# ChenFengYe/motion-latent-diffusion

Hardware: NVIDIA H100
Metric: motions/sec @ 50-step DDIM text-to-motion, batch 256 (higher is better)
Workload: dtype f16x2-split (fp32-equivalent, fp32 accumulate)

## Files before the change

### mld_b200/csrc/engine.cu

```cuda
#include "engine.h"

#include <math.h>
#include <string.h>

#include <algorithm>

#include "gemm_tc.h"
#include "misc_kernels.cuh"

static thread_local std::string g_err;
void mldb_set_err(const std::string& s) { g_err = s; }
extern "C" const char* mldb_last_error(void) { return g_err.c_str(); }
extern "C" int mldb_abi_version(void) { return MLDB_ABI_VERSION; }

extern "C" void mldb_default_config(mldb_config* c) {
  memset(c, 0, sizeof *c);
  c->abi_version = MLDB_ABI_VERSION;
  c->cond_kind = MLDB_COND_TEXT;
  c->arch = MLDB_ARCH_TRANS_ENC;
  c->latent_dim = 256; c->n_lat = 1; c->num_heads = 4; c->ff_size = 1024; c->num_layers = 9;
  c->text_dim = 768; c->nclasses = 12; c->nfeats = 263; c->diffusion_only = 0;
  c->flip_sin_to_cos = 1; c->freq_shift = 0.0f; c->guidance_scale = 7.5f;
  c->vae_kind = MLDB_VAE_MLD; c->vae_layers = 9; c->vae_heads = 4; c->vae_ff = 1024;
  c->vae_nfeats = 263;
// ... 379 lines not shown
  env = getenv("MLDB_BRANCHES");
  if (env) h->branches = std::min(std::max(atoi(env), 1), (int)mldb_handle::MAX_BRANCHES);
  e = cudaEventCreateWithFlags(&h->ev_fork, cudaEventDisableTiming);
  for (int i = 0; i < mldb_handle::MAX_BRANCHES - 1 && e == cudaSuccess; ++i) {
    e = cudaStreamCreateWithFlags(&h->br_stream[i], cudaStreamNonBlocking);
    if (e == cudaSuccess) e = cudaEventCreateWithFlags(&h->ev_join[i], cudaEventDisableTiming);
  }
  if (e != cudaSuccess) { mldb_destroy(h); FAIL(MLDB_ERR_CUDA, "branch streams: %s", cudaGetErrorString(e)); }
  for (int i = 0; i < mldb_handle::MAX_BRANCHES && e == cudaSuccess; ++i) {
    e = cudaMalloc((void**)&h->ffn_scratch[i], TC_FFN_SCRATCH_BYTES);
    if (e == cudaSuccess) e = cudaMalloc((void**)&h->ffn_flags[i], TC_FFN_FLAG_BYTES);
    if (e == cudaSuccess) e = cudaMemset(h->ffn_flags[i], 0, TC_FFN_FLAG_BYTES);
  }
  if (e != cudaSuccess) { mldb_destroy(h); FAIL(MLDB_ERR_CUDA, "ffn scratch: %s", cudaGetErrorString(e)); }
  env = getenv("MLDB_FFN_SPLIT");
  if (env) tc_set_ffn_split(h->tc, atoi(env) != 0);
  env = getenv("MLDB_FFN_FUSED");
  if (env) tc_set_ffn_fused(h->tc, atoi(env) != 0);
  *out = h;
  return MLDB_OK;
}

extern "C" void mldb_destroy(mldb_handle* h) {
  if (!h) return;
  DeviceGuard guard(h->device);
  cudaDeviceSynchronize();
  for (auto& kv : h->plans) {
    if (kv.second->exec) cudaGraphExecDestroy(kv.second->exec);
    delete kv.second;
  }
  for (void* p : h->allocs) cudaFree(p);
  if (h->cap_stream) cudaStreamDestroy(h->cap_stream);
  for (int i = 0; i < mldb_handle::MAX_BRANCHES - 1; ++i) {
    if (h->br_stream[i]) cudaStreamDestroy(h->br_stream[i]);
    if (h->ev_join[i]) cudaEventDestroy(h->ev_join[i]);
  }
  if (h->ev_fork) cudaEventDestroy(h->ev_fork);
  for (int i = 0; i < mldb_handle::MAX_BRANCHES; ++i) { cudaFree(h->ffn_scratch[i]); cudaFree(h->ffn_flags[i]); }
  mldb_comm_release(h);
  tc_destroy(h->tc);
  delete h;
}

extern "C" int mldb_set_option(mldb_handle* h, const char* name, const char* value) {
  if (!h || !name || !value) FAIL(MLDB_ERR_INVALID, "null argument");
  if (!strcmp(name, "gemm")) {
    if (!strcmp(value, "tc")) h->use_tc = true;
    else if (!strcmp(value, "simt")) h->use_tc = false;
    else FAIL(MLDB_ERR_INVALID, "gemm must be tc|simt");
  } else if (!strcmp(name, "ffn_fused")) {
    tc_set_ffn_fused(h->tc, atoi(value) != 0);
  } else if (!strcmp(name, "ffn_split")) {
    tc_set_ffn_split(h->tc, atoi(value) != 0);
  } else if (!strcmp(name, "attn")) {
    if (!strcmp(value, "tc")) h->attn_kind = 0;
    else if (!strcmp(value, "mma")) h->attn_kind = 1;
    else if (!strcmp(value, "simt")) h->attn_kind = 2;
    else FAIL(MLDB_ERR_INVALID, "attn must be tc|mma|simt");
  } else if (!strcmp(name, "branches")) {
    h->branches = std::min(std::max(atoi(value), 1), (int)mldb_handle::MAX_BRANCHES);
  } else if (!strcmp(name, "graph")) {
    h->use_graph = strcmp(value, "0") != 0;
  } else if (!strcmp(name, "t2m_chunk")) {
    h->t2m.chunk = std::max(atoi(value), 0);
  } else if (!strcmp(name, "a2m_chunk")) {
    h->a2m.chunk = std::max(atoi(value), 0);
  } else if (!strcmp(name, "stgcn_chunk")) {
    h->stgcn.chunk = std::max(atoi(value), 0);
  } else if (!strcmp(name, "smpl_chunk")) {
    h->smpl.chunk = std::max(atoi(value), 0);
  } else {
    FAIL(MLDB_ERR_INVALID, "unknown option %s", name);
  }
  for (auto& kv : h->plans) {
    if (kv.second->exec) { cudaGraphExecDestroy(kv.second->exec); kv.second->exec = nullptr; }
  }
  return MLDB_OK;
}

extern "C" int64_t mldb_launch_count(const mldb_handle* h) { return h ? h->launches : 0; }

extern "C" int mldb_load_tensor(mldb_handle* h, const char* key, const void* data,
                                const int64_t* shape, int32_t ndim, int32_t dtype) {
  if (!h || !key || !data || (!shape && ndim != 0)) FAIL(MLDB_ERR_INVALID, "null argument");
  if (dtype != MLDB_DTYPE_F32) FAIL(MLDB_ERR_UNSUPPORTED, "only fp32 tensors are accepted");
  if (h->finalized) FAIL(MLDB_ERR_STATE, "weights already finalized");
  auto it = h->raw.find(key);
  if (it == h->raw.end()) FAIL(MLDB_ERR_INVALID, "unexpected state-dict key '%s'", key);
  RawTensor& t = it->second;
  if ((int)t.shape.size() != ndim) FAIL(MLDB_ERR_INVALID, "key '%s': rank %d, expected %d", key, ndim, (int)t.shape.size());
  size_t n = 1;
  for (int i = 0; i < ndim; ++i) {
    if (shape[i] != t.shape[i]) FAIL(MLDB_ERR_INVALID, "key '%s': dim %d is %lld, expected %lld", key, i, (long long)shape[i], (long long)t.shape[i]);
    n *= (size_t)shape[i];
  }
  t.host.resize(n);
  DeviceGuard guard(h->device);
  CK(cudaMemcpy(t.host.data(), data, n * sizeof(float), cudaMemcpyDefault));
  t.loaded = true;
  return MLDB_OK;
}

extern "C" int mldb_finalize_weights(mldb_handle* h, void* stream) {
  (void)stream;
  if (!h) FAIL(MLDB_ERR_INVALID, "null handle");
  if (h->finalized) FAIL(MLDB_ERR_STATE, "already finalized");
// ... 228 lines not shown
```

### mld_b200/csrc/gemm_tc.cu

```cuda
#include "gemm_tc.h"

#include <algorithm>

#include "tc_common.cuh"

namespace {
using namespace tc;

constexpr int BM = 128, BK = 64;
constexpr int NUM_THREADS = 384;
constexpr int MMA_THREADS = 256;
constexpr int CONSUMER_WARPS = 8;
constexpr int MAX_N = 1024;
constexpr int MAX_N_WIDE = 4096;

struct TcParams {
  int M, N, kblocks, kb1;
  int m_tiles, n_tiles;
  float inv_scale;
  const float* bias;
  const float* addtab;
  int act;
  __half* out_hi; __half* out_lo; int ld_out, out_col0;
  float* out_f32; int ldc;
  const float* res_f32;
  int in_group, out_group, out_off;
  const int32_t* zero_lengths;
  const __half* res_hi; const __half* res_lo; int ld_res;
  const float* gamma; const float* beta;
  long long* tl;
};

enum { EPI_FAST = 0, EPI_LN = 1, EPI_GENERIC = 2, EPI_RES = 3, EPI_F32 = 4 };

template <int BN>
struct TileCfg {
  static constexpr int A_BYTES = BM * BK * 2;
  static constexpr int W_BYTES = BN * BK * 2;
  static constexpr int STAGE_BYTES = 2 * A_BYTES + 2 * W_BYTES;
  static constexpr int STAGES = BN == 256 ? 2 : 3;
  static constexpr int SMEM_BYTES = STAGES * STAGE_BYTES + 256 + 1024;
  static_assert(SMEM_BYTES <= 232448, "shared memory budget");
};

__device__ __forceinline__ void store_split2(__half* hi, __half* lo, int64_t o, float x0, float x1) {
  uint32_t h, l;
  split2(x0, x1, h, l);
  *reinterpret_cast<uint32_t*>(hi + o) = h;
  *reinterpret_cast<uint32_t*>(lo + o) = l;
}

template <int ACT, int N>
__device__ __forceinline__ void fast_group(const float (&d)[N], int j, float sc, float2 b, float (&x)[4]) {
  x[0] = fmaf(d[4 * j], sc, b.x); x[1] = fmaf(d[4 * j + 1], sc, b.y);
  x[2] = fmaf(d[4 * j + 2], sc, b.x); x[3] = fmaf(d[4 * j + 3], sc, b.y);
#pragma unroll
  for (int e = 0; e < 4; ++e) {
    if (ACT == ACT_GELU) x[e] = gelu_fast(x[e]);
    if (ACT == ACT_QUICKGELU) x[e] = quick_gelu_f(x[e]);
    if (ACT == ACT_LEAKY) x[e] = apply_act(x[e], ACT_LEAKY);
  }
}

__device__ __forceinline__ void quad_transpose(uint32_t (&v)[4], int l) {
  const bool b2 = l & 2, b1 = l & 1;
  uint32_t r0 = __shfl_xor_sync(0xffffffffu, b2 ? v[0] : v[2], 2), r1 = __shfl_xor_sync(0xffffffffu, b2 ? v[1] : v[3], 2);
  if (b2) { v[0] = r0; v[1] = r1; } else { v[2] = r0; v[3] = r1; }
  r0 = __shfl_xor_sync(0xffffffffu, b1 ? v[0] : v[1], 1); r1 = __shfl_xor_sync(0xffffffffu, b1 ? v[2] : v[3], 1);
  if (b1) { v[0] = r0; v[2] = r1; } else { v[1] = r0; v[3] = r1; }
}

template <class Load>
__device__ __forceinline__ void ring_produce(int& q_next, int total, int need, const uint64_t* bar_empty, int stages,
                                             Load&& load) {
  while (q_next < total) {
    const uint32_t bar = smem_u32(&bar_empty[q_next % stages]), par = (((uint32_t)(q_next / stages)) & 1u) ^ 1u;
    if (q_next <= need) mbar_wait(bar, par);
    else if (!__shfl_sync(0xffffffffu, (int)mbar_test(bar, par), 0)) break;
    load(q_next++);
  }
}

template <class Res, class Out>
__device__ __forceinline__ void ln_rows(float (&d)[128], float sc, const float* bias, const float* gamma,
                                        const float* beta, int cp, Res&& res, Out&& out) {
  float s0 = 0.0f, s1 = 0.0f;
#pragma unroll
  for (int j = 0; j < 32; ++j) {
    const int n = 8 * j + cp;
    const float2 b = bias ? __ldg(reinterpret_cast<const float2*>(bias + n)) : make_float2(0.0f, 0.0f);
    float x[4] = {fmaf(d[4 * j], sc, b.x), fmaf(d[4 * j + 1], sc, b.y), fmaf(d[4 * j + 2], sc, b.x),
                  fmaf(d[4 * j + 3], sc, b.y)};
    res(j, x);
    d[4 * j] = x[0]; d[4 * j + 1] = x[1]; d[4 * j + 2] = x[2]; d[4 * j + 3] = x[3];
    s0 += x[0] + x[1]; s1 += x[2] + x[3];
  }
  const float mean0 = quad_sum(s0) * (1.0f / 256), mean1 = quad_sum(s1) * (1.0f / 256);
  float q0 = 0.0f, q1 = 0.0f;
#pragma unroll
  for (int j = 0; j < 32; ++j) {
    const float a0 = d[4 * j] - mean0, a1 = d[4 * j + 1] - mean0, a2 = d[4 * j + 2] - mean1, a3 = d[4 * j + 3] - mean1;
    d[4 * j] = a0; d[4 * j + 1] = a1; d[4 * j + 2] = a2; d[4 * j + 3] = a3;
    q0 = fmaf(a0, a0, fmaf(a1, a1, q0));
    q1 = fmaf(a2, a2, fmaf(a3, a3, q1));
  }
  const float rstd0 = rsqrtf(quad_sum(q0) * (1.0f / 256) + 1e-5f), rstd1 = rsqrtf(quad_sum(q1) * (1.0f / 256) + 1e-5f);
#pragma unroll
  for (int j = 0; j < 32; ++j) {
    const int n = 8 * j + cp;
    const float2 g = __ldg(reinterpret_cast<const float2*>(gamma + n)), be = __ldg(reinterpret_cast<const float2*>(beta + n));
    const float y[4] = {fmaf(d[4 * j] * rstd0, g.x, be.x), fmaf(d[4 * j + 1] * rstd0, g.y, be.y),
                        fmaf(d[4 * j + 2] * rstd1, g.x, be.x), fmaf(d[4 * j + 3] * rstd1, g.y, be.y)};
    out(j, y);
  }
}

__device__ __forceinline__ void ln_epilogue(float (&d)[128], float sc, const float* bias, const __half* res_hi,
                                            const __half* res_lo, int ld_res, const float* gamma, const float* beta,
                                            __half* out_hi, __half* out_lo, int ld_out, int r_lo, int M, int cp) {
  const bool ok0 = r_lo < M, ok1 = r_lo + 8 < M;
  ln_rows(d, sc, bias, gamma, beta, cp,
          [&](int j, float (&x)[4]) {
            if (!res_hi) return;
            const int n = 8 * j + cp;
            if (ok0) {
              const int64_t o = (int64_t)r_lo * ld_res + n;
              const float2 h = __half22float2(*reinterpret_cast<const __half2*>(res_hi + o));
              const float2 l = __half22float2(*reinterpret_cast<const __half2*>(res_lo + o));
              x[0] = (x[0] + h.x) + l.x; x[1] = (x[1] + h.y) + l.y;
            }
            if (ok1) {
              const int64_t o = (int64_t)(r_lo + 8) * ld_res + n;
              const float2 h = __half22float2(*reinterpret_cast<const __half2*>(res_hi + o));
              const float2 l = __half22float2(*reinterpret_cast<const __half2*>(res_lo + o));
              x[2] = (x[2] + h.x) + l.x; x[3] = (x[3] + h.y) + l.y;
            }
          },
          [&](int j, const float (&y)[4]) {
            const int n = 8 * j + cp;
            if (ok0) store_split2(out_hi, out_lo, (int64_t)r_lo * ld_out + n, y[0], y[1]);
            if (ok1) store_split2(out_hi, out_lo, (int64_t)(r_lo + 8) * ld_out + n, y[2], y[3]);
          });
}

__device__ __forceinline__ void ln_tile(float (&d)[128], float sc, const float* bias, const float* gamma,
                                        const float* beta, uint8_t* tile, int rl, int lane, int cp) {
  uint8_t* const row0 = tile + rl * 128 + cp * 2;
  const int sw = lane >> 2;
  auto at = [&](int j, int h, int plane) {
    return reinterpret_cast<__half2*>(row0 + plane * 65536 + h * 1024 + (j >> 3) * 16384 + (((j & 7) ^ sw) << 4));
  };
  ln_rows(d, sc, bias, gamma, beta, cp,
          [&](int j, float (&x)[4]) {
#pragma unroll
            for (int h = 0; h < 2; ++h) {
              const float2 hi = __half22float2(*at(j, h, 0)), lo = __half22float2(*at(j, h, 1));
              x[2 * h] = (x[2 * h] + hi.x) + lo.x; x[2 * h + 1] = (x[2 * h + 1] + hi.y) + lo.y;
            }
          },
          [&](int j, const float (&y)[4]) {
#pragma unroll
            for (int h = 0; h < 2; ++h) {
              uint32_t hi, lo;
              split2(y[2 * h], y[2 * h + 1], hi, lo);
              *reinterpret_cast<uint32_t*>(at(j, h, 0)) = hi;
              *reinterpret_cast<uint32_t*>(at(j, h, 1)) = lo;
            }
          });
}

template <int BN, int EPI, int ACT = ACT_NONE>
__global__ void __launch_bounds__(NUM_THREADS, 1)
k_gemm_tc(const __grid_constant__ CUtensorMap tmA1h, const __grid_constant__ CUtensorMap tmA1l,
          const __grid_constant__ CUtensorMap tmA2h, const __grid_constant__ CUtensorMap tmA2l,
          const __grid_constant__ CUtensorMap tmWh, const __grid_constant__ CUtensorMap tmWl, const TcParams p) {
  static_assert(EPI != EPI_LN || BN == 256, "the LayerNorm epilogue covers a full 256-wide row");
  using Cfg = TileCfg<BN>;
  constexpr int STAGES = Cfg::STAGES;
  extern __shared__ uint8_t smem_raw[];
  uint8_t* smem = smem_raw + smem_pad1024(smem_raw);
  uint64_t* bar_full = reinterpret_cast<uint64_t*>(smem + STAGES * Cfg::STAGE_BYTES);
  uint64_t* bar_empty = bar_full + STAGES;

  const int warp = __shfl_sync(0xffffffffu, (int)(threadIdx.x >> 5), 0), lane = threadIdx.x & 31;
  int tl_n = 0;
  tl_event(p.tl, tl_n, 40);
  const int ntiles = p.m_tiles * p.n_tiles;
  const int nlocal = (ntiles - (int)blockIdx.x + (int)gridDim.x - 1) / (int)gridDim.x;
  auto decode = [&](int j, int& m0, int& n0) {
    const int t = (int)blockIdx.x + j * (int)gridDim.x;
    m0 = (t / p.n_tiles) * BM;
    n0 = (t % p.n_tiles) * BN;
  };

  if (threadIdx.x == 0) {
    for (int s = 0; s < STAGES; ++s) {
      mbar_init(smem_u32(&bar_full[s]), 1);
      mbar_init(smem_u32(&bar_empty[s]), CONSUMER_WARPS);
    }
    asm volatile("fence.mbarrier_init.release.cluster;" ::: "memory");
    tma_prefetch_desc(&tmA1h); tma_prefetch_desc(&tmA1l); tma_prefetch_desc(&tmWh); tma_prefetch_desc(&tmWl);
  }
  pdl_trigger();
  __syncthreads();
  pdl_wait();
  tl_event(p.tl, tl_n, 41);

  if (warp < 4) {
    reg_dec<40>();
    if (warp != 0) return;
    int kbg = 0;
    for (int j = 0; j < nlocal; ++j) {
      int m0, n0;
      decode(j, m0, n0);
      tl_event(p.tl, tl_n, 1, j);
      for (int kb = 0; kb < p.kblocks; ++kb, ++kbg) {
        const int s = kbg % STAGES;
        mbar_wait(smem_u32(&bar_empty[s]), (((uint32_t)(kbg / STAGES)) & 1u) ^ 1u);
        if (elect_one()) {
          if (kb == 0 && j + 1 < nlocal) {
            int m1, n1;
            decode(j + 1, m1, n1);
            if (m1 != m0) {
              for (int k2 = 0; k2 < p.kblocks; ++k2) {
                if (k2 < p.kb1) { tma_prefetch_2d(&tmA1h, k2 * BK, m1); tma_prefetch_2d(&tmA1l, k2 * BK, m1); }
                else { tma_prefetch_2d(&tmA2h, (k2 - p.kb1) * BK, m1); tma_prefetch_2d(&tmA2l, (k2 - p.kb1) * BK, m1); }
              }
            }
          }
          const uint32_t full = smem_u32(&bar_full[s]);
          mbar_expect_tx(full, Cfg::STAGE_BYTES);
          const uint32_t sAh = smem_u32(smem + s * Cfg::STAGE_BYTES), sAl = sAh + Cfg::A_BYTES;
          const uint32_t sWh = sAl + Cfg::A_BYTES, sWl = sWh + Cfg::W_BYTES;
          if (kb < p.kb1) {
            tma_load_2d(sAh, &tmA1h, full, kb * BK, m0);
            tma_load_2d(sAl, &tmA1l, full, kb * BK, m0);
          } else {
            tma_load_2d(sAh, &tmA2h, full, (kb - p.kb1) * BK, m0);
            tma_load_2d(sAl, &tmA2l, full, (kb - p.kb1) * BK, m0);
          }
          tma_load_2d(sWh, &tmWh, full, kb * BK, n0);
          tma_load_2d(sWl, &tmWl, full, kb * BK, n0);
        }
        __syncwarp();
      }
    }
    return;
  }
  reg_inc<232>();
  const int cw = (warp >> 2) - 1;
  const int cp = 2 * (lane & 3);
  float d[BN / 2];
  int kbg = 0;
  for (int it = 0; it < nlocal; ++it) {
    int m0, n0;
    decode(it, m0, n0);
    tl_event(p.tl, tl_n, 2, it);
    for (int kb = 0; kb < p.kblocks; ++kb, ++kbg) {
      const int s = kbg % STAGES;
      mbar_wait(smem_u32(&bar_full[s]), ((uint32_t)(kbg / STAGES)) & 1u);
      const uint32_t sAh = smem_u32(smem + s * Cfg::STAGE_BYTES) + cw * (64 * 128), sAl = sAh + Cfg::A_BYTES;
      const uint32_t sWh = smem_u32(smem + s * Cfg::STAGE_BYTES) + 2 * Cfg::A_BYTES, sWl = sWh + Cfg::W_BYTES;
      wg_fence();
      kblock_ss<BN>(d, sAh, sAl, sWh, sWl, kb == 0);
      wg_commit();
      if (kb > 0) {
        wg_wait<1>();
        if (lane == 0) mbar_arrive(smem_u32(&bar_empty[(kbg - 1) % STAGES]));
      }
    }
    wg_wait<0>();
    acc_fence(d);
    if (lane == 0) mbar_arrive(smem_u32(&bar_empty[(kbg - 1) % STAGES]));
    tl_event(p.tl, tl_n, 4, it);

    const int r_lo = m0 + cw * 64 + (warp & 3) * 16 + (lane >> 2);
    if constexpr (EPI == EPI_LN) {
      ln_epilogue(d, p.inv_scale, p.bias, p.res_hi, p.res_lo, p.ld_res, p.gamma, p.beta, p.out_hi, p.out_lo, p.ld_out,
                  r_lo, p.M, cp);
    } else if constexpr (EPI == EPI_FAST) {
      const bool ok0 = r_lo < p.M, ok1 = r_lo + 8 < p.M;
      const int64_t o0 = (int64_t)r_lo * p.ld_out + p.out_col0 + n0 + cp, o1 = o0 + (int64_t)8 * p.ld_out;
#pragma unroll
      for (int j = 0; j < BN / 8; ++j) {
        float x[4];
        fast_group<ACT>(d, j, p.inv_scale, __ldg(reinterpret_cast<const float2*>(p.bias + n0 + 8 * j + cp)), x);
        if (ok0) store_split2(p.out_hi, p.out_lo, o0 + 8 * j, x[0], x[1]);
        if (ok1) store_split2(p.out_hi, p.out_lo, o1 + 8 * j, x[2], x[3]);
      }
    } else if constexpr (EPI == EPI_RES) {
      const float sc = p.inv_scale;
#pragma unroll
      for (int j = 0; j < BN / 8; ++j) {
        const int n = n0 + 8 * j + cp;
        if (n >= p.N) continue;
        const float2 b = p.bias ? __ldg(reinterpret_cast<const float2*>(p.bias + n)) : make_float2(0.0f, 0.0f);
#pragma unroll
        for (int h = 0; h < 2; ++h) {
          if (r_lo + 8 * h >= p.M) continue;
          const int64_t o = (int64_t)(r_lo + 8 * h) * p.ldc + n;
          const float2 r = *reinterpret_cast<const float2*>(p.res_f32 + o);
          *reinterpret_cast<float2*>(p.out_f32 + o) =
              make_float2(fmaf(d[4 * j + 2 * h], sc, b.x) + r.x, fmaf(d[4 * j + 2 * h + 1], sc, b.y) + r.y);
        }
      }
    } else if constexpr (EPI == EPI_F32) {
      const float sc = p.inv_scale;
#pragma unroll
      for (int j = 0; j < BN / 8; ++j) {
        const int n = n0 + 8 * j + cp;
        if (n >= p.N) continue;
        const float2 b = p.bias ? __ldg(reinterpret_cast<const float2*>(p.bias + n)) : make_float2(0.0f, 0.0f);
#pragma unroll
        for (int h = 0; h < 2; ++h) {
          if (r_lo + 8 * h >= p.M) continue;
          const float x0 = apply_act(fmaf(d[4 * j + 2 * h], sc, b.x), ACT), x1 = apply_act(fmaf(d[4 * j + 2 * h + 1], sc, b.y), ACT);
          *reinterpret_cast<float2*>(p.out_f32 + (int64_t)(r_lo + 8 * h) * p.ldc + n) = make_float2(x0, x1);
        }
      }
    } else {
#pragma unroll
      for (int h = 0; h < 2; ++h) {
        const int m = r_lo + 8 * h;
        if (m >= p.M) continue;
        int seq = 0, pos = m;
        if (p.in_group < p.M) { seq = m / p.in_group; pos = m - seq * p.in_group; }
        const int64_t orow = (int64_t)seq * p.out_group + p.out_off + pos;
        const bool zero = p.zero_lengths != nullptr && pos >= p.zero_lengths[seq];
        const float* tab = p.addtab ? p.addtab + (int64_t)(p.out_off + pos) * p.N : nullptr;
#pragma unroll
        for (int j = 0; j < BN / 8; ++j) {
#pragma unroll
// ... 461 lines not shown
    tl_event(p.tl, tl_n, 53, i);
  };
  auto step = [&](int i, float (&cur)[64], float (&prev)[64]) {
    const bool fresh = first_of_tile(i);
    const int j = tile_of(i);
    tl_event(p.tl, tl_n, 50, i);
#pragma unroll
    for (int k = 0; k < 4; ++k) {
      const int q = 4 * i + k;
      if (warp == 0) produce(q, fresh ? 4 * j + k : -1);
      if (fresh) {
        mbar_wait(smem_u32(&bar_afull[k]), (uint32_t)j & 1u);
        if (k == 0) tl_event(p.tl, tl_n, 51, j);
      }
      mbar_wait(smem_u32(&bar_full[q % STAGES]), ((uint32_t)(q / STAGES)) & 1u);
      const uint32_t w = smem_u32(ring + (q % STAGES) * Cfg::STAGE_BYTES), a = sA + k * 16384;
      wg_fence();
      kblock_ss<128>(cur, a, a + 65536, w, w + Cfg::STAGE_BYTES / 2, k == 0);
      wg_commit();
      if (k == 2) {
        if (warp == 0) produce(q + 1, -1);
        if (i > 0) epilogue(prev, i - 1);
      }
      if (q > 0) {
        wg_wait<1>();
        retire(q - 1);
      }
      if (k == 0 && i > 0) acc_fence(prev);
    }
  };
  for (int i = 0; i < n; i += 2) {
    step(i, acc0, acc1);
    if (i + 1 < n) step(i + 1, acc1, acc0);
  }
  wg_wait<0>();
  retire(4 * n - 1);
  if ((n - 1) & 1) {
    acc_fence(acc1);
    epilogue(acc1, n - 1);
  } else {
    acc_fence(acc0);
    epilogue(acc0, n - 1);
  }
  tl_event(p.tl, tl_n, 42);
}

}

struct TcCtx {
  int device = 0;
  int sm_count = 132;
  int ffn_fused = 1;
  int ffn_split = 1;
};

TcCtx* tc_create(int device) {
  if (!tc::tmap_encoder()) return nullptr;
  TcCtx* c = new TcCtx();
  c->device = device;
  cudaDeviceGetAttribute(&c->sm_count, cudaDevAttrMultiProcessorCount, device);
  bool ok = true;
  auto opt_in = [&](auto kernel, int bytes) { ok = ok && smem_opt_in(kernel, bytes, "k_gemm_tc"); };
  opt_in(k_gemm_tc<256, EPI_FAST>, TileCfg<256>::SMEM_BYTES); opt_in(k_gemm_tc<128, EPI_FAST>, TileCfg<128>::SMEM_BYTES);
  opt_in(k_gemm_tc<256, EPI_FAST, ACT_GELU>, TileCfg<256>::SMEM_BYTES); opt_in(k_gemm_tc<128, EPI_FAST, ACT_GELU>, TileCfg<128>::SMEM_BYTES);
  opt_in(k_gemm_tc<256, EPI_GENERIC>, TileCfg<256>::SMEM_BYTES); opt_in(k_gemm_tc<128, EPI_GENERIC>, TileCfg<128>::SMEM_BYTES);
  opt_in(k_gemm_tc<256, EPI_FAST, ACT_QUICKGELU>, TileCfg<256>::SMEM_BYTES);
  opt_in(k_gemm_tc<128, EPI_FAST, ACT_QUICKGELU>, TileCfg<128>::SMEM_BYTES);
  opt_in(k_gemm_tc<256, EPI_RES>, TileCfg<256>::SMEM_BYTES); opt_in(k_gemm_tc<128, EPI_RES>, TileCfg<128>::SMEM_BYTES);
  opt_in(k_gemm_tc<256, EPI_LN>, TileCfg<256>::SMEM_BYTES);
  opt_in(k_gemm_tc<256, EPI_FAST, ACT_LEAKY>, TileCfg<256>::SMEM_BYTES); opt_in(k_gemm_tc<128, EPI_FAST, ACT_LEAKY>, TileCfg<128>::SMEM_BYTES);
  opt_in(k_gemm_tc<256, EPI_F32>, TileCfg<256>::SMEM_BYTES); opt_in(k_gemm_tc<128, EPI_F32>, TileCfg<128>::SMEM_BYTES);
  opt_in(k_gemm_tc<256, EPI_F32, ACT_LEAKY>, TileCfg<256>::SMEM_BYTES); opt_in(k_gemm_tc<128, EPI_F32, ACT_LEAKY>, TileCfg<128>::SMEM_BYTES);
  opt_in(k_ffn_tc, FfnCfg::SMEM_BYTES);
  opt_in(k_proj_tc<ACT_NONE>, ProjCfg::SMEM_BYTES); opt_in(k_proj_tc<ACT_GELU>, ProjCfg::SMEM_BYTES);
  opt_in(k_proj_tc<ACT_QUICKGELU>, ProjCfg::SMEM_BYTES); opt_in(k_proj_tc<ACT_LEAKY>, ProjCfg::SMEM_BYTES);
  if (!ok) {
    delete c;
    return nullptr;
  }
  return c;
}
void tc_destroy(TcCtx* c) { delete c; }

static int pick_bn(const GemmArgs& g) { return (g.w.N % 256 == 0) ? 256 : 128; }

bool tc_gemm_supported(const TcCtx* c, const GemmArgs& g) {
  if (!c) return false;
  if (g.a_kind != A_SPLIT || g.M < 1 || g.w.N > (g.wide_n ? MAX_N_WIDE : MAX_N)) return false;
  if (g.K1 <= 0 || g.K1 % BK || g.K2 % BK || g.a1.cols != g.K1) return false;
  if (g.K2 > 0 && g.a2.cols != g.K2) return false;
  if (g.w.K != g.K1 + g.K2) return false;
  if (((uintptr_t)g.a1.hi & 15) || ((uintptr_t)g.w.w & 15)) return false;
  if (g.out.hi && ((g.out.cols % 8) || (g.out_col0 % 8))) return false;
  if (g.res_f32 && (!g.out_f32 || g.out.hi || g.act != ACT_NONE || g.addtab || g.zero_lengths || g.in_group < g.M ||
                    g.out_group != 0 || g.out_off != 0 || (g.w.N % 2) || (g.ldc % 2) || ((uintptr_t)g.out_f32 & 7) ||
                    ((uintptr_t)g.res_f32 & 7)))
    return false;
  return true;
}

bool tc_gemm_ln_supported(const TcCtx* c, const GemmArgs& g, const LnArgs& l) {
  if (!tc_gemm_supported(c, g)) return false;
  if (g.w.N != 256 || l.d != 256 || g.act != ACT_NONE) return false;
  if (l.in_group != 0 || l.c != nullptr || l.out_f32 != nullptr || !l.out.hi) return false;
  if (l.out.cols != 256 || (l.res.hi && l.res.cols != 256)) return false;
  if (l.gamma2 || l.rowvec) return false;
  if (g.addtab || g.zero_lengths || g.in_group < g.M || g.out_group != 0 || g.out_off != 0) return false;
  return true;
}

static void fill_params(const GemmArgs& g, const LnArgs* ln, int bn, TcParams* out) {
  TcParams p{};
  p.M = g.M; p.N = g.w.N; p.kblocks = g.w.K / BK; p.kb1 = g.K1 / BK;
  p.inv_scale = g.w.inv_scale; p.bias = g.w.bias; p.addtab = g.addtab; p.act = g.act;
  p.in_group = g.in_group; p.out_group = g.out_group; p.out_off = g.out_off; p.zero_lengths = g.zero_lengths;
  if (ln) {
    p.out_hi = ln->out.hi; p.out_lo = ln->out.lo(); p.ld_out = ln->out.cols; p.out_col0 = 0;
    p.res_hi = ln->res.hi; p.res_lo = ln->res.hi ? ln->res.lo() : nullptr; p.ld_res = ln->res.cols;
    p.gamma = ln->gamma; p.beta = ln->beta;
  } else {
    p.out_hi = g.out.hi; p.out_lo = g.out.hi ? g.out.lo() : nullptr; p.ld_out = g.out.cols; p.out_col0 = g.out_col0;
    p.out_f32 = g.out_f32; p.ldc = g.ldc; p.res_f32 = g.res_f32;
  }
  p.m_tiles = (g.M + BM - 1) / BM;
  p.n_tiles = (g.w.N + bn - 1) / bn;
  p.tl = tc::mldb_timeline_buffer();
  *out = p;
}

static bool tc_proj(TcCtx* c, const GemmArgs& g, cudaStream_t st) {
  CUtensorMap mAh, mAl, mWh, mWl;
  const bool ok = make_map(&mAh, g.a1.hi, g.M, g.K1, BM) && make_map(&mAl, g.a1.lo(), g.M, g.K1, BM) &&
                  make_map(&mWh, g.w.w, g.w.N, g.w.K, ProjCfg::CHUNK) &&
                  make_map(&mWl, g.w.w + g.w.plane_stride, g.w.N, g.w.K, ProjCfg::CHUNK);
  if (!ok) return false;
  ProjParams p{};
  p.M = g.M; p.n_chunks = g.w.N / ProjCfg::CHUNK; p.items = (g.M + BM - 1) / BM * p.n_chunks;
  p.inv_scale = g.w.inv_scale; p.bias = g.w.bias;
  p.out_hi = g.out.hi; p.out_lo = g.out.lo(); p.ld_out = g.out.cols; p.out_col0 = g.out_col0;
  p.tl = tc::mldb_timeline_buffer();
  const dim3 grid(p.items < c->sm_count ? p.items : c->sm_count);
  switch (g.act) {
    case ACT_GELU: launch_pdl(k_proj_tc<ACT_GELU>, grid, dim3(MMA_THREADS), ProjCfg::SMEM_BYTES, st, mAh, mAl, mWh, mWl, p); break;
    case ACT_QUICKGELU: launch_pdl(k_proj_tc<ACT_QUICKGELU>, grid, dim3(MMA_THREADS), ProjCfg::SMEM_BYTES, st, mAh, mAl, mWh, mWl, p); break;
    case ACT_LEAKY: launch_pdl(k_proj_tc<ACT_LEAKY>, grid, dim3(MMA_THREADS), ProjCfg::SMEM_BYTES, st, mAh, mAl, mWh, mWl, p); break;
    default: launch_pdl(k_proj_tc<ACT_NONE>, grid, dim3(MMA_THREADS), ProjCfg::SMEM_BYTES, st, mAh, mAl, mWh, mWl, p); break;
  }
  return true;
}

bool tc_gemm(TcCtx* c, const GemmArgs& g, const LnArgs* ln, cudaStream_t st) {
  const int bn = ln ? 256 : pick_bn(g);
  const bool fast = !ln && g.out.hi && !g.out_f32 && !g.addtab && !g.zero_lengths && g.in_group >= g.M &&
                    g.out_group == 0 && g.out_off == 0 && g.w.N % bn == 0 && g.w.bias != nullptr &&
                    (g.act == ACT_NONE || g.act == ACT_GELU || g.act == ACT_QUICKGELU || g.act == ACT_LEAKY);
  if (fast && g.K1 == 256 && g.K2 == 0 && ((uintptr_t)g.out.hi & 15) == 0 && ((uintptr_t)g.out.lo() & 15) == 0)
    return tc_proj(c, g, st);
  CUtensorMap mA1h, mA1l, mA2h, mA2l, mWh, mWl;
  bool ok = make_map(&mA1h, g.a1.hi, g.M, g.K1, BM) && make_map(&mA1l, g.a1.lo(), g.M, g.K1, BM);
  if (g.K2 > 0) ok = ok && make_map(&mA2h, g.a2.hi, g.M, g.K2, BM) && make_map(&mA2l, g.a2.lo(), g.M, g.K2, BM);
  else { mA2h = mA1h; mA2l = mA1l; }
  ok = ok && make_map(&mWh, g.w.w, g.w.N, g.w.K, bn) && make_map(&mWl, g.w.w + g.w.plane_stride, g.w.N, g.w.K, bn);
  if (!ok) return false;
  TcParams p;
  fill_params(g, ln, bn, &p);
  const bool f32 = !ln && g.vec_f32 && !g.out.hi && g.out_f32 && !g.res_f32 && !g.addtab && !g.zero_lengths &&
                   g.in_group >= g.M && g.out_group == 0 && g.out_off == 0 && g.w.N % 2 == 0 && g.ldc % 2 == 0 &&
                   ((uintptr_t)g.out_f32 & 7) == 0 && (g.act == ACT_NONE || g.act == ACT_LEAKY);
  const int ntiles = p.m_tiles * p.n_tiles;
  dim3 grid(ntiles < c->sm_count ? ntiles : c->sm_count);
#define MLDB_LAUNCH(BN_, ...)                                                                                      \
  launch_pdl(k_gemm_tc<BN_, __VA_ARGS__>, grid, dim3(NUM_THREADS), TileCfg<BN_>::SMEM_BYTES, st, mA1h, mA1l, mA2h, \
             mA2l, mWh, mWl, p)
#define MLDB_LAUNCH_SHAPE(...)                                                       \
  do {                                                                               \
    if (bn == 256) MLDB_LAUNCH(256, __VA_ARGS__); else MLDB_LAUNCH(128, __VA_ARGS__); \
  } while (0)
  if (ln)                             MLDB_LAUNCH(256, EPI_LN);
  else if (g.res_f32)                 MLDB_LAUNCH_SHAPE(EPI_RES);
  else if (fast && g.act == ACT_GELU) MLDB_LAUNCH_SHAPE(EPI_FAST, ACT_GELU);
  else if (fast && g.act == ACT_QUICKGELU) MLDB_LAUNCH_SHAPE(EPI_FAST, ACT_QUICKGELU);
  else if (fast && g.act == ACT_LEAKY) MLDB_LAUNCH_SHAPE(EPI_FAST, ACT_LEAKY);
  else if (f32 && g.act == ACT_LEAKY) MLDB_LAUNCH_SHAPE(EPI_F32, ACT_LEAKY);
  else if (f32)                       MLDB_LAUNCH_SHAPE(EPI_F32);
  else if (fast)                      MLDB_LAUNCH_SHAPE(EPI_FAST);
  else                                MLDB_LAUNCH_SHAPE(EPI_GENERIC);
#undef MLDB_LAUNCH_SHAPE
#undef MLDB_LAUNCH
  return true;
}

int tc_set_ffn_split(TcCtx* c, int on) {
  if (!c) return 0;
  const int old = c->ffn_split;
  c->ffn_split = on;
  return old;
}
int tc_set_ffn_fused(TcCtx* c, int on) {
  if (!c) return 0;
  const int old = c->ffn_fused;
  c->ffn_fused = on;
  return old;
}
static bool planes_aligned16(const ActBuf& b) { return ((uintptr_t)b.hi & 15) == 0 && ((uintptr_t)b.lo() & 15) == 0; }

bool tc_ffn_supported(const TcCtx* c, const GemmArgs& g1, const GemmArgs& g2, const LnArgs& l2) {
  if (!c || !c->ffn_fused) return false;
  if (!tc_gemm_supported(c, g1) || !tc_gemm_ln_supported(c, g2, l2)) return false;
  if (g1.K1 != 256 || g1.K2 > 0 || g2.K2 > 0 || g1.M != g2.M) return false;
  if (g1.w.N % FfnCfg::CHUNK || g1.w.N > MAX_N || g1.w.N != g2.K1) return false;
  if (g1.act != ACT_GELU || g1.out_f32 || g1.addtab || g1.zero_lengths) return false;
  if (g1.in_group < g1.M || g1.out_group != 0 || g1.out_off != 0) return false;
  if (l2.res.hi != g1.a1.hi || l2.res.plane_stride != g1.a1.plane_stride) return false;
  if (!planes_aligned16(g1.a1) || !planes_aligned16(l2.out)) return false;
  return true;
}
bool tc_tail_supported(const TcCtx* c, const GemmArgs& go, const LnArgs& l1, const GemmArgs& g1, const GemmArgs& g2,
                       const LnArgs& l2) {
  if (!tc_gemm_ln_supported(c, go, l1) || !tc_ffn_supported(c, g1, g2, l2)) return false;
  if (go.K1 != 256 || go.K2 > 0 || go.M != g1.M || !l1.res.hi) return false;
  if (g1.a1.hi != l1.out.hi || g1.a1.plane_stride != l1.out.plane_stride) return false;
  return planes_aligned16(go.a1) && planes_aligned16(l1.res);
}

static bool launch_ffn(TcCtx* c, const GemmArgs* go, const LnArgs* l1, const GemmArgs& g1, const GemmArgs& g2,
                       const LnArgs& l2, float* scratch, int* flags, cudaStream_t st) {
  CUtensorMap mXh, mXl, mW1h, mW1l, mW2h, mW2l, mAh, mAl, mWoh, mWol, mYh, mYl;
  const int M = g1.M, m_tiles = (M + BM - 1) / BM;
  const ActBuf x = go ? l1->res : g1.a1;
  bool ok = make_map(&mXh, x.hi, M, 256, BM) && make_map(&mXl, x.lo(), M, 256, BM) &&
            make_map(&mW1h, g1.w.w, g1.w.N, g1.w.K, FfnCfg::CHUNK) &&
            make_map(&mW1l, g1.w.w + g1.w.plane_stride, g1.w.N, g1.w.K, FfnCfg::CHUNK) &&
            make_map(&mW2h, g2.w.w, g2.w.N, g2.w.K, 256) &&
            make_map(&mW2l, g2.w.w + g2.w.plane_stride, g2.w.N, g2.w.K, 256) &&
            make_map(&mYh, l2.out.hi, M, 256, 64) && make_map(&mYl, l2.out.lo(), M, 256, 64);
  if (go) {
    ok = ok && make_map(&mAh, go->a1.hi, M, 256, BM) && make_map(&mAl, go->a1.lo(), M, 256, BM) &&
         make_map(&mWoh, go->w.w, go->w.N, go->w.K, 256) && make_map(&mWol, go->w.w + go->w.plane_stride, go->w.N, go->w.K, 256);
  } else {
    mAh = mXh; mAl = mXl; mWoh = mW2h; mWol = mW2l;
  }
  if (!ok) return false;
  FfnParams p{};
  p.M = M; p.m_tiles = m_tiles; p.n_chunks = g1.w.N / FfnCfg::CHUNK;
  p.tl = tc::mldb_timeline_buffer();
  p.prefix = go ? 1 : 0;
  if (go) { p.inv_s0 = go->w.inv_scale; p.b0 = go->w.bias; p.gamma1 = l1->gamma; p.beta1 = l1->beta; }
  p.inv_s1 = g1.w.inv_scale; p.inv_s2 = g2.w.inv_scale;
  p.b1 = g1.w.bias; p.b2 = g2.w.bias; p.gamma = l2.gamma; p.beta = l2.beta;
  const int ncta_max = c->sm_count;
  p.full = m_tiles / ncta_max; p.left = m_tiles % ncta_max; p.parts = 1;
  p.scratch = scratch; p.flags = flags;
  if (p.left > 0 && scratch && flags && c->ffn_split) {
    const int parts = std::min(p.n_chunks, ncta_max / p.left);
    if (parts >= 2 && (size_t)p.left * (parts - 1) * (BM * 256 * 4) <= TC_FFN_SCRATCH_BYTES) p.parts = parts;
  }
  const int ncta = p.full > 0 ? ncta_max : p.left * p.parts;
// ... 13 lines not shown
```

### mld_b200/csrc/gemm_tc.h

```cpp
#pragma once
#include "ops.cuh"

struct TcCtx;
TcCtx* tc_create(int device);
void tc_destroy(TcCtx* c);
bool tc_gemm_supported(const TcCtx* c, const GemmArgs& g);
bool tc_gemm_ln_supported(const TcCtx* c, const GemmArgs& g, const LnArgs& l);
bool tc_gemm(TcCtx* c, const GemmArgs& g, const LnArgs* ln, cudaStream_t st);
bool tc_ffn_supported(const TcCtx* c, const GemmArgs& g1, const GemmArgs& g2, const LnArgs& l2);
constexpr size_t TC_FFN_SCRATCH_BYTES = (size_t)160 * 128 * 256 * 4, TC_FFN_FLAG_BYTES = 160 * 4;
bool tc_ffn(TcCtx* c, const GemmArgs& g1, const GemmArgs& g2, const LnArgs& l2, float* scratch, int* flags, cudaStream_t st);
bool tc_tail_supported(const TcCtx* c, const GemmArgs& go, const LnArgs& l1, const GemmArgs& g1, const GemmArgs& g2,
                       const LnArgs& l2);
bool tc_tail(TcCtx* c, const GemmArgs& go, const LnArgs& l1, const GemmArgs& g1, const GemmArgs& g2, const LnArgs& l2,
             float* scratch, int* flags, cudaStream_t st);
int tc_set_ffn_split(TcCtx* c, int on);
int tc_set_ffn_fused(TcCtx* c, int on);
```

### mld_b200/csrc/tc_common.cuh

```cuda
#pragma once
#include <cuda.h>
#include <stdio.h>
#include <stdlib.h>
#include <string.h>

#include <string>

#include "common.cuh"

namespace tc {

__device__ __forceinline__ uint32_t smem_u32(const void* p) { return (uint32_t)__cvta_generic_to_shared(p); }
__device__ __forceinline__ uint32_t smem_pad1024(const void* raw) { return (1024u - (smem_u32(raw) & 1023u)) & 1023u; }

__device__ __forceinline__ void mbar_init(uint32_t bar, uint32_t count) {
  asm volatile("mbarrier.init.shared::cta.b64 [%0], %1;" ::"r"(bar), "r"(count) : "memory");
}
__device__ __forceinline__ void mbar_expect_tx(uint32_t bar, uint32_t bytes) {
  asm volatile("mbarrier.arrive.expect_tx.shared::cta.b64 _, [%0], %1;" ::"r"(bar), "r"(bytes) : "memory");
}
__device__ __forceinline__ void mbar_arrive(uint32_t bar) {
  asm volatile("mbarrier.arrive.shared::cta.b64 _, [%0];" ::"r"(bar) : "memory");
}
__device__ __forceinline__ void mbar_arrive_cnt(uint32_t bar, uint32_t n) {
// ... 2 lines not shown
__device__ __forceinline__ void mbar_wait(uint32_t bar, uint32_t parity) {
  uint32_t done = 0, spins = 0;
  long long t0 = 0;
  do {
    asm volatile(
        "{\n\t.reg .pred p;\n\t"
        "mbarrier.try_wait.parity.shared::cta.b64 p, [%1], %2;\n\t"
        "selp.u32 %0, 1, 0, p;\n\t}"
        : "=r"(done)
        : "r"(bar), "r"(parity)
        : "memory");
    if (!done && (++spins & 1023u) == 0) {
      const long long now = clock64();
      if (t0 == 0) t0 = now;
      else if (now - t0 > 4000000000ll) __trap();
    }
  } while (!done);
}
__device__ __forceinline__ bool mbar_test(uint32_t bar, uint32_t parity) {
  uint32_t done;
  asm volatile(
      "{\n\t.reg .pred p;\n\t"
      "mbarrier.test_wait.parity.shared::cta.b64 p, [%1], %2;\n\t"
      "selp.u32 %0, 1, 0, p;\n\t}"
      : "=r"(done)
      : "r"(bar), "r"(parity)
      : "memory");
  return done != 0;
}

__device__ __forceinline__ void tma_load_2d(uint32_t dst, const CUtensorMap* map, uint32_t bar, int c0, int c1) {
  asm volatile(
      "cp.async.bulk.tensor.2d.shared::cluster.global.mbarrier::complete_tx::bytes [%0], [%1, {%3, %4}], [%2];"
      ::"r"(dst), "l"(reinterpret_cast<uint64_t>(map)), "r"(bar), "r"(c0), "r"(c1)
      : "memory");
}
__device__ __forceinline__ void tma_load_3d(uint32_t dst, const CUtensorMap* map, uint32_t bar, int c0, int c1, int c2) {
  asm volatile(
      "cp.async.bulk.tensor.3d.shared::cluster.global.mbarrier::complete_tx::bytes [%0], [%1, {%3, %4, %5}], [%2];"
      ::"r"(dst), "l"(reinterpret_cast<uint64_t>(map)), "r"(bar), "r"(c0), "r"(c1), "r"(c2)
      : "memory");
}
__device__ __forceinline__ void tma_load_4d(uint32_t dst, const CUtensorMap* map, uint32_t bar, int c0, int c1, int c2,
                                            int c3) {
  asm volatile(
      "cp.async.bulk.tensor.4d.shared::cluster.global.mbarrier::complete_tx::bytes [%0], [%1, {%3, %4, %5, %6}], [%2];"
      ::"r"(dst), "l"(reinterpret_cast<uint64_t>(map)), "r"(bar), "r"(c0), "r"(c1), "r"(c2), "r"(c3)
      : "memory");
}
__device__ __forceinline__ void tma_prefetch_2d(const CUtensorMap* map, int c0, int c1) {
  asm volatile("cp.async.bulk.prefetch.tensor.2d.L2.global.tile [%0, {%1, %2}];"
               ::"l"(reinterpret_cast<uint64_t>(map)), "r"(c0), "r"(c1) : "memory");
}
__device__ __forceinline__ void tma_prefetch_desc(const CUtensorMap* map) {
  asm volatile("prefetch.tensormap [%0];" ::"l"(reinterpret_cast<uint64_t>(map)) : "memory");
}
__device__ __forceinline__ void tma_store_2d(const CUtensorMap* map, uint32_t src, int c0, int c1) {
  asm volatile("cp.async.bulk.tensor.2d.global.shared::cta.bulk_group [%0, {%2, %3}], [%1];"
               ::"l"(reinterpret_cast<uint64_t>(map)), "r"(src), "r"(c0), "r"(c1) : "memory");
}
__device__ __forceinline__ void bulk_commit() { asm volatile("cp.async.bulk.commit_group;" ::: "memory"); }
template <int N> __device__ __forceinline__ void bulk_wait_read() {
  asm volatile("cp.async.bulk.wait_group.read %0;" ::"n"(N) : "memory");
}
__device__ __forceinline__ void fence_async_smem() { asm volatile("fence.proxy.async.shared::cta;" ::: "memory"); }

__device__ __forceinline__ bool elect_one() {
  uint32_t pred;
  asm volatile("{\n\t.reg .pred p;\n\telect.sync _|p, 0xffffffff;\n\tselp.u32 %0, 1, 0, p;\n\t}" : "=r"(pred));
  return pred != 0;
}

template <int N> __device__ __forceinline__ void reg_dec() { asm volatile("setmaxnreg.dec.sync.aligned.u32 %0;" ::"n"(N)); }
template <int N> __device__ __forceinline__ void reg_inc() { asm volatile("setmaxnreg.inc.sync.aligned.u32 %0;" ::"n"(N)); }
__device__ __forceinline__ void named_bar_sync(int id, int threads) {
  asm volatile("bar.sync %0, %1;" ::"r"(id), "r"(threads) : "memory");
}

__device__ __forceinline__ void wg_fence() { asm volatile("wgmma.fence.sync.aligned;" ::: "memory"); }
__device__ __forceinline__ void wg_commit() { asm volatile("wgmma.commit_group.sync.aligned;" ::: "memory"); }
template <int N> __device__ __forceinline__ void wg_wait() { asm volatile("wgmma.wait_group.sync.aligned %0;" ::"n"(N) : "memory"); }

template <int N> __device__ __forceinline__ void acc_fence(float (&d)[N]) {
#pragma unroll
  for (int i = 0; i < N; ++i) asm volatile("" : "+f"(d[i])::"memory");
}

__device__ __forceinline__ uint64_t make_desc(uint32_t saddr) {
  return (uint64_t)((saddr >> 4) & 0x3FFF) | ((uint64_t)1 << 16) | ((uint64_t)(1024 >> 4) << 32) | ((uint64_t)1 << 62);
}
__device__ __forceinline__ void wgmma_ss_n256(float (&d)[128], uint64_t adesc, uint64_t bdesc, uint32_t acc) {
  asm volatile(
      "{\n\t.reg .pred p;\n\t"
      "setp.ne.b32 p, %130, 0;\n\t"
      "wgmma.mma_async.sync.aligned.m64n256k16.f32.f16.f16 "
      "{%0, %1, %2, %3, %4, %5, %6, %7, %8, %9, %10, %11, %12, %13, %14, %15, "
      "%16, %17, %18, %19, %20, %21, %22, %23, %24, %25, %26, %27, %28, %29, %30, %31, "
      "%32, %33, %34, %35, %36, %37, %38, %39, %40, %41, %42, %43, %44, %45, %46, %47, "
      "%48, %49, %50, %51, %52, %53, %54, %55, %56, %57, %58, %59, %60, %61, %62, %63, "
      "%64, %65, %66, %67, %68, %69, %70, %71, %72, %73, %74, %75, %76, %77, %78, %79, "
      "%80, %81, %82, %83, %84, %85, %86, %87, %88, %89, %90, %91, %92, %93, %94, %95, "
      "%96, %97, %98, %99, %100, %101, %102, %103, %104, %105, %106, %107, %108, %109, %110, %111, "
      "%112, %113, %114, %115, %116, %117, %118, %119, %120, %121, %122, %123, %124, %125, %126, %127}, "
      "%128, %129, p, 1, 1, 0, 0;\n\t}"
      : "+f"(d[0]), "+f"(d[1]), "+f"(d[2]), "+f"(d[3]), "+f"(d[4]), "+f"(d[5]), "+f"(d[6]), "+f"(d[7]),
        "+f"(d[8]), "+f"(d[9]), "+f"(d[10]), "+f"(d[11]), "+f"(d[12]), "+f"(d[13]), "+f"(d[14]), "+f"(d[15]),
// ... 231 lines not shown
```

Measured before the change: 839.0.

## Vectorize LN epilogue residual loads and stores with quad transposes, prefetch residual to L2

The LayerNorm GEMM epilogue now handles columns in groups of four. Each lane issues 16-byte loads and stores, and quad shuffles transpose the data between the MMA fragment layout and a contiguous row layout. This replaces many 4-byte scattered accesses. The producer warp also issues bulk L2 prefetches of the residual rows for the current and next tile. A runtime toggle and alignment checks gate the path, and it adds shuffle overhead and register pressure in exchange.

Measured after the change: 830.7, median of 6. No clear change (-1.0%).

```diff
diff --git a/mld_b200/csrc/engine.cu b/mld_b200/csrc/engine.cu
--- a/mld_b200/csrc/engine.cu
+++ b/mld_b200/csrc/engine.cu
@@ -455,6 +455,8 @@
     tc_set_ffn_fused(h->tc, atoi(value) != 0);
   } else if (!strcmp(name, "ffn_split")) {
     tc_set_ffn_split(h->tc, atoi(value) != 0);
+  } else if (!strcmp(name, "ln_vec")) {
+    tc_set_ln_vec(h->tc, atoi(value) != 0);
   } else if (!strcmp(name, "attn")) {
     if (!strcmp(value, "tc")) h->attn_kind = 0;
     else if (!strcmp(value, "mma")) h->attn_kind = 1;
diff --git a/mld_b200/csrc/gemm_tc.cu b/mld_b200/csrc/gemm_tc.cu
--- a/mld_b200/csrc/gemm_tc.cu
+++ b/mld_b200/csrc/gemm_tc.cu
@@ -28,6 +28,7 @@
   const int32_t* zero_lengths;
   const __half* res_hi; const __half* res_lo; int ld_res;
   const float* gamma; const float* beta;
+  int ln_vec;
   long long* tl;
 };
 
@@ -62,6 +63,8 @@
   }
 }
 
+__device__ __forceinline__ int nctaid_x() { int n; asm volatile("mov.u32 %0, %%nctaid.x;" : "=r"(n)); return n; }
+
 __device__ __forceinline__ void quad_transpose(uint32_t (&v)[4], int l) {
   const bool b2 = l & 2, b1 = l & 1;
   uint32_t r0 = __shfl_xor_sync(0xffffffffu, b2 ? v[0] : v[2], 2), r1 = __shfl_xor_sync(0xffffffffu, b2 ? v[1] : v[3], 2);
@@ -81,19 +84,22 @@
   }
 }
 
-template <class Res, class Out>
+template <int G, class Res, class Out>
 __device__ __forceinline__ void ln_rows(float (&d)[128], float sc, const float* bias, const float* gamma,
                                         const float* beta, int cp, Res&& res, Out&& out) {
   float s0 = 0.0f, s1 = 0.0f;
 #pragma unroll
-  for (int j = 0; j < 32; ++j) {
-    const int n = 8 * j + cp;
-    const float2 b = bias ? __ldg(reinterpret_cast<const float2*>(bias + n)) : make_float2(0.0f, 0.0f);
-    float x[4] = {fmaf(d[4 * j], sc, b.x), fmaf(d[4 * j + 1], sc, b.y), fmaf(d[4 * j + 2], sc, b.x),
-                  fmaf(d[4 * j + 3], sc, b.y)};
-    res(j, x);
-    d[4 * j] = x[0]; d[4 * j + 1] = x[1]; d[4 * j + 2] = x[2]; d[4 * j + 3] = x[3];
-    s0 += x[0] + x[1]; s1 += x[2] + x[3];
+  for (int jb = 0; jb < 32 / G; ++jb) {
+#pragma unroll
+    for (int j = G * jb; j < G * jb + G; ++j) {
+      const int n = 8 * j + cp;
+      const float2 b = bias ? __ldg(reinterpret_cast<const float2*>(bias + n)) : make_float2(0.0f, 0.0f);
+      d[4 * j] = fmaf(d[4 * j], sc, b.x); d[4 * j + 1] = fmaf(d[4 * j + 1], sc, b.y);
+      d[4 * j + 2] = fmaf(d[4 * j + 2], sc, b.x); d[4 * j + 3] = fmaf(d[4 * j + 3], sc, b.y);
+    }
+    res(jb, d);
+#pragma unroll
+    for (int j = G * jb; j < G * jb + G; ++j) { s0 += d[4 * j] + d[4 * j + 1]; s1 += d[4 * j + 2] + d[4 * j + 3]; }
   }
   const float mean0 = quad_sum(s0) * (1.0f / 256), mean1 = quad_sum(s1) * (1.0f / 256);
   float q0 = 0.0f, q1 = 0.0f;
@@ -106,40 +112,80 @@
   }
   const float rstd0 = rsqrtf(quad_sum(q0) * (1.0f / 256) + 1e-5f), rstd1 = rsqrtf(quad_sum(q1) * (1.0f / 256) + 1e-5f);
 #pragma unroll
-  for (int j = 0; j < 32; ++j) {
-    const int n = 8 * j + cp;
-    const float2 g = __ldg(reinterpret_cast<const float2*>(gamma + n)), be = __ldg(reinterpret_cast<const float2*>(beta + n));
-    const float y[4] = {fmaf(d[4 * j] * rstd0, g.x, be.x), fmaf(d[4 * j + 1] * rstd0, g.y, be.y),
-                        fmaf(d[4 * j + 2] * rstd1, g.x, be.x), fmaf(d[4 * j + 3] * rstd1, g.y, be.y)};
-    out(j, y);
+  for (int jb = 0; jb < 32 / G; ++jb) {
+    float y[4 * G];
+#pragma unroll
+    for (int g = 0; g < G; ++g) {
+      const int j = G * jb + g, n = 8 * j + cp;
+      const float2 ga = __ldg(reinterpret_cast<const float2*>(gamma + n)), be = __ldg(reinterpret_cast<const float2*>(beta + n));
+      y[4 * g] = fmaf(d[4 * j] * rstd0, ga.x, be.x); y[4 * g + 1] = fmaf(d[4 * j + 1] * rstd0, ga.y, be.y);
+      y[4 * g + 2] = fmaf(d[4 * j + 2] * rstd1, ga.x, be.x); y[4 * g + 3] = fmaf(d[4 * j + 3] * rstd1, ga.y, be.y);
+    }
+    out(jb, y);
   }
 }
 
 __device__ __forceinline__ void ln_epilogue(float (&d)[128], float sc, const float* bias, const __half* res_hi,
                                             const __half* res_lo, int ld_res, const float* gamma, const float* beta,
-                                            __half* out_hi, __half* out_lo, int ld_out, int r_lo, int M, int cp) {
+                                            __half* out_hi, __half* out_lo, int ld_out, int r_lo, int M, int lane,
+                                            bool vec) {
+  const int l = lane & 3, cp = 2 * l;
   const bool ok0 = r_lo < M, ok1 = r_lo + 8 < M;
-  ln_rows(d, sc, bias, gamma, beta, cp,
-          [&](int j, float (&x)[4]) {
+  ln_rows<4>(d, sc, bias, gamma, beta, cp,
+          [&](int jb, float (&x)[128]) {
             if (!res_hi) return;
-            const int n = 8 * j + cp;
-            if (ok0) {
-              const int64_t o = (int64_t)r_lo * ld_res + n;
-              const float2 h = __half22float2(*reinterpret_cast<const __half2*>(res_hi + o));
-              const float2 l = __half22float2(*reinterpret_cast<const __half2*>(res_lo + o));
-              x[0] = (x[0] + h.x) + l.x; x[1] = (x[1] + h.y) + l.y;
-            }
-            if (ok1) {
-              const int64_t o = (int64_t)(r_lo + 8) * ld_res + n;
-              const float2 h = __half22float2(*reinterpret_cast<const __half2*>(res_hi + o));
-              const float2 l = __half22float2(*reinterpret_cast<const __half2*>(res_lo + o));
-              x[2] = (x[2] + h.x) + l.x; x[3] = (x[3] + h.y) + l.y;
+#pragma unroll
+            for (int h = 0; h < 2; ++h) {
+              const bool ok = h ? ok1 : ok0;
+              const int64_t o = (int64_t)(r_lo + 8 * h) * ld_res;
+              uint32_t wh[4] = {}, wl[4] = {};
+              if (vec) {
+                if (ok) {
+                  const uint4 vh = *reinterpret_cast<const uint4*>(res_hi + o + 32 * jb + 8 * l);
+                  const uint4 vl = *reinterpret_cast<const uint4*>(res_lo + o + 32 * jb + 8 * l);
+                  wh[0] = vh.x; wh[1] = vh.y; wh[2] = vh.z; wh[3] = vh.w;
+                  wl[0] = vl.x; wl[1] = vl.y; wl[2] = vl.z; wl[3] = vl.w;
+                }
+                quad_transpose(wh, l); quad_transpose(wl, l);
+              } else if (ok) {
+#pragma unroll
+                for (int g = 0; g < 4; ++g) {
+                  wh[g] = *reinterpret_cast<const uint32_t*>(res_hi + o + 8 * (4 * jb + g) + cp);
+                  wl[g] = *reinterpret_cast<const uint32_t*>(res_lo + o + 8 * (4 * jb + g) + cp);
+                }
+              }
+              if (!ok) continue;
+#pragma unroll
+              for (int g = 0; g < 4; ++g) {
+                const float2 hf = __half22float2(*reinterpret_cast<const __half2*>(&wh[g]));
+                const float2 lf = __half22float2(*reinterpret_cast<const __half2*>(&wl[g]));
+                float* const e = x + 16 * jb + 4 * g + 2 * h;
+                e[0] = (e[0] + hf.x) + lf.x; e[1] = (e[1] + hf.y) + lf.y;
+              }
             }
           },
-          [&](int j, const float (&y)[4]) {
-            const int n = 8 * j + cp;
-            if (ok0) store_split2(out_hi, out_lo, (int64_t)r_lo * ld_out + n, y[0], y[1]);
-            if (ok1) store_split2(out_hi, out_lo, (int64_t)(r_lo + 8) * ld_out + n, y[2], y[3]);
+          [&](int jb, const float (&y)[16]) {
+#pragma unroll
+            for (int h = 0; h < 2; ++h) {
+              const bool ok = h ? ok1 : ok0;
+              const int64_t o = (int64_t)(r_lo + 8 * h) * ld_out;
+              uint32_t wh[4], wl[4];
+#pragma unroll
+              for (int g = 0; g < 4; ++g) split2(y[4 * g + 2 * h], y[4 * g + 2 * h + 1], wh[g], wl[g]);
+              if (vec) {
+                quad_transpose(wh, l); quad_transpose(wl, l);
+                if (ok) {
+                  *reinterpret_cast<uint4*>(out_hi + o + 32 * jb + 8 * l) = make_uint4(wh[0], wh[1], wh[2], wh[3]);
+                  *reinterpret_cast<uint4*>(out_lo + o + 32 * jb + 8 * l) = make_uint4(wl[0], wl[1], wl[2], wl[3]);
+                }
+              } else if (ok) {
+#pragma unroll
+                for (int g = 0; g < 4; ++g) {
+                  *reinterpret_cast<uint32_t*>(out_hi + o + 8 * (4 * jb + g) + cp) = wh[g];
+                  *reinterpret_cast<uint32_t*>(out_lo + o + 8 * (4 * jb + g) + cp) = wl[g];
+                }
+              }
+            }
           });
 }
 
@@ -150,12 +196,12 @@
   auto at = [&](int j, int h, int plane) {
     return reinterpret_cast<__half2*>(row0 + plane * 65536 + h * 1024 + (j >> 3) * 16384 + (((j & 7) ^ sw) << 4));
   };
-  ln_rows(d, sc, bias, gamma, beta, cp,
-          [&](int j, float (&x)[4]) {
+  ln_rows<1>(d, sc, bias, gamma, beta, cp,
+          [&](int j, float (&x)[128]) {
 #pragma unroll
             for (int h = 0; h < 2; ++h) {
               const float2 hi = __half22float2(*at(j, h, 0)), lo = __half22float2(*at(j, h, 1));
-              x[2 * h] = (x[2 * h] + hi.x) + lo.x; x[2 * h + 1] = (x[2 * h + 1] + hi.y) + lo.y;
+              x[4 * j + 2 * h] = (x[4 * j + 2 * h] + hi.x) + lo.x; x[4 * j + 2 * h + 1] = (x[4 * j + 2 * h + 1] + hi.y) + lo.y;
             }
           },
           [&](int j, const float (&y)[4]) {
@@ -188,7 +234,7 @@
   const int ntiles = p.m_tiles * p.n_tiles;
   const int nlocal = (ntiles - (int)blockIdx.x + (int)gridDim.x - 1) / (int)gridDim.x;
   auto decode = [&](int j, int& m0, int& n0) {
-    const int t = (int)blockIdx.x + j * (int)gridDim.x;
+    const int t = (int)blockIdx.x + j * nctaid_x();
     m0 = (t / p.n_tiles) * BM;
     n0 = (t % p.n_tiles) * BN;
   };
@@ -213,11 +259,24 @@
     for (int j = 0; j < nlocal; ++j) {
       int m0, n0;
       decode(j, m0, n0);
-      tl_event(p.tl, tl_n, 1, j);
       for (int kb = 0; kb < p.kblocks; ++kb, ++kbg) {
         const int s = kbg % STAGES;
         mbar_wait(smem_u32(&bar_empty[s]), (((uint32_t)(kbg / STAGES)) & 1u) ^ 1u);
         if (elect_one()) {
+          if (EPI == EPI_LN && kb == 0 && p.ln_vec && p.res_hi) {
+            auto pf = [&](int m) {
+              const int64_t o = (int64_t)m * p.ld_res;
+              const uint32_t bytes = (uint32_t)(min(BM, p.M - m) * p.ld_res * 2);
+              bulk_prefetch_l2(p.res_hi + o, bytes);
+              bulk_prefetch_l2(p.res_lo + o, bytes);
+            };
+            if (j == 0) pf(m0);
+            if (j + 1 < nlocal) {
+              int m1, n1;
+              decode(j + 1, m1, n1);
+              pf(m1);
+            }
+          }
           if (kb == 0 && j + 1 < nlocal) {
             int m1, n1;
             decode(j + 1, m1, n1);
@@ -277,7 +336,7 @@
     const int r_lo = m0 + cw * 64 + (warp & 3) * 16 + (lane >> 2);
     if constexpr (EPI == EPI_LN) {
       ln_epilogue(d, p.inv_scale, p.bias, p.res_hi, p.res_lo, p.ld_res, p.gamma, p.beta, p.out_hi, p.out_lo, p.ld_out,
-                  r_lo, p.M, cp);
+                  r_lo, p.M, lane, p.ln_vec != 0);
     } else if constexpr (EPI == EPI_FAST) {
       const bool ok0 = r_lo < p.M, ok1 = r_lo + 8 < p.M;
       const int64_t o0 = (int64_t)r_lo * p.ld_out + p.out_col0 + n0 + cp, o1 = o0 + (int64_t)8 * p.ld_out;
@@ -845,6 +904,7 @@
   int sm_count = 132;
   int ffn_fused = 1;
   int ffn_split = 1;
+  int ln_vec = 1;
 };
 
 TcCtx* tc_create(int device) {
@@ -875,6 +935,8 @@
 }
 void tc_destroy(TcCtx* c) { delete c; }
 
+static bool planes_aligned16(const ActBuf& b) { return ((uintptr_t)b.hi & 15) == 0 && ((uintptr_t)b.lo() & 15) == 0; }
+
 static int pick_bn(const GemmArgs& g) { return (g.w.N % 256 == 0) ? 256 : 128; }
 
 bool tc_gemm_supported(const TcCtx* c, const GemmArgs& g) {
@@ -957,6 +1019,10 @@
   if (!ok) return false;
   TcParams p;
   fill_params(g, ln, bn, &p);
+  if (ln) {
+    const bool res_ok = !ln->res.hi || (planes_aligned16(ln->res) && ln->res.cols % 8 == 0);
+    p.ln_vec = c->ln_vec && res_ok && planes_aligned16(ln->out) && ln->out.cols % 8 == 0;
+  }
   const bool f32 = !ln && g.vec_f32 && !g.out.hi && g.out_f32 && !g.res_f32 && !g.addtab && !g.zero_lengths &&
                    g.in_group >= g.M && g.out_group == 0 && g.out_off == 0 && g.w.N % 2 == 0 && g.ldc % 2 == 0 &&
                    ((uintptr_t)g.out_f32 & 7) == 0 && (g.act == ACT_NONE || g.act == ACT_LEAKY);
@@ -989,13 +1055,18 @@
   c->ffn_split = on;
   return old;
 }
+int tc_set_ln_vec(TcCtx* c, int on) {
+  if (!c) return 0;
+  const int old = c->ln_vec;
+  c->ln_vec = on;
+  return old;
+}
 int tc_set_ffn_fused(TcCtx* c, int on) {
   if (!c) return 0;
   const int old = c->ffn_fused;
   c->ffn_fused = on;
   return old;
 }
-static bool planes_aligned16(const ActBuf& b) { return ((uintptr_t)b.hi & 15) == 0 && ((uintptr_t)b.lo() & 15) == 0; }
 
 bool tc_ffn_supported(const TcCtx* c, const GemmArgs& g1, const GemmArgs& g2, const LnArgs& l2) {
   if (!c || !c->ffn_fused) return false;
diff --git a/mld_b200/csrc/gemm_tc.h b/mld_b200/csrc/gemm_tc.h
--- a/mld_b200/csrc/gemm_tc.h
+++ b/mld_b200/csrc/gemm_tc.h
@@ -16,3 +16,4 @@
              float* scratch, int* flags, cudaStream_t st);
 int tc_set_ffn_split(TcCtx* c, int on);
 int tc_set_ffn_fused(TcCtx* c, int on);
+int tc_set_ln_vec(TcCtx* c, int on);
diff --git a/mld_b200/csrc/tc_common.cuh b/mld_b200/csrc/tc_common.cuh
--- a/mld_b200/csrc/tc_common.cuh
+++ b/mld_b200/csrc/tc_common.cuh
@@ -78,6 +78,9 @@
   asm volatile("cp.async.bulk.prefetch.tensor.2d.L2.global.tile [%0, {%1, %2}];"
                ::"l"(reinterpret_cast<uint64_t>(map)), "r"(c0), "r"(c1) : "memory");
 }
+__device__ __forceinline__ void bulk_prefetch_l2(const void* p, uint32_t bytes) {
+  asm volatile("cp.async.bulk.prefetch.L2.global [%0], %1;" ::"l"(p), "r"(bytes) : "memory");
+}
 __device__ __forceinline__ void tma_prefetch_desc(const CUtensorMap* map) {
   asm volatile("prefetch.tensormap [%0];" ::"l"(reinterpret_cast<uint64_t>(map)) : "memory");
 }
```
